# cvxgrp/qcqp

Measured on AMD Instinct MI355X. Metric: restarts x coord-sweeps / sec (improve COORD_DESCENT phase-2 sweeps, 2n^2 flops each; whole step timed), higher is better.
Workload: dtype f64

## Files before the change

### qcqp_amd/csrc/capi.hip

```cpp
#include <dlfcn.h>
#include <unistd.h>
#include <hip/hip_runtime.h>
#include <rccl/rccl.h>

#include <algorithm>
#include <cmath>
#include <cstdarg>
#include <cstdio>
#include <cstring>
#include <string>
#include <chrono>
#include <vector>

#include "../../include/qcqp_mi.h"
#include "kernels_impl.h"
#include "admm.h"
#include "admm_fused.h"
#include "cd_queue.h"
#include "cd_life.h"
#include "cd_small.h"
#include "sdr_small.h"
#include "gemm_pk.h"
#include "cd_general.h"
#include "cd_dense.h"
// ... 131 lines not shown
    double stream_limit = 16e9;
    double *dn_gp_pre = nullptr, *dn_tmp = nullptr;
    ncclComm_t comm = nullptr;
    int rank = 0, world = 1;
    double *d_comm = nullptr, *d_comm_big = nullptr;
    int64_t comm_big_cap = 0;
    long long *d_prof = nullptr;
    int cd_stage = 0;
    int64_t Xi_cap = 0;
    bool sdr_factor_resident = false;
    double ad_Minv_rho = 0.0;
    bool ad_Minv_device = false;
    const char *last_cd2_kernel = "";
    bool profile = false;
    int dbg = 0;
    char *af_work = nullptr;
    size_t af_work_cap = 0;
    bool ad_fused = true;
    int ad_fused_nt = 512;
    const char *last_admm_kernel = "";
    int last_admm_C = 0;
    long long af_prof[16] = {0};
    int cd_queue = 2;
    int *d_qnext = nullptr;
    bool q_prepared = false;
    CdLife *d_life = nullptr;
    int Kreal = 0;
    double fbound = 0.0;
    double *l2_scratch = nullptr; size_t l2_scratch_cap = 0;
    double *l2_D = nullptr, *l2_S = nullptr;
    int *l2_abort = nullptr;
    int *l2_cuslot = nullptr;
    double *l2_preslack = nullptr; int64_t l2_preslack_cap = 0;
    double *lr_L = nullptr, *lr_G = nullptr, *lr_U = nullptr; int lr_RB = 0;
    int life_version = 0;
    long long *d_life_prof = nullptr;
    int64_t *d_bestK_idx = nullptr; double *d_bestK_key = nullptr, *d_bestK_x = nullptr; int64_t bestK_cap = 0;
    bool cd_ref_order = false;
    bool force_generic = false;
    std::vector<int> last_st1, last_st2;
    char *sb_work = nullptr;
    size_t sb_work_cap = 0;
    std::vector<double> unit_d;
    char *ss_work = nullptr;
    size_t ss_work_cap = 0;
};

namespace {

void admm_free(qcqpmi_ctx *c, bool keep_zsolver);

int fail(qcqpmi_ctx *c, int code, const char *fmt, ...) {
    char buf[1024];
    va_list ap;
    va_start(ap, fmt);
    vsnprintf(buf, sizeof(buf), fmt, ap);
    va_end(ap);
    if (c) c->err = buf; else g_create_error = buf;
    return code;
}

#define HIPCHK(c, expr)                                                                       \
    do {                                                                                      \
        hipError_t e_ = (expr);                                                               \
        if (e_ != hipSuccess)                                                                 \
            return fail(c, QCQPMI_EHIP, "%s failed: %s (%s:%d)", #expr, hipGetErrorString(e_), \
// ... 463 lines not shown
    if (!out || n <= 0 || m < 0) return fail(nullptr, QCQPMI_EINVAL, "ctx_create: bad arguments");
    int ndev = qcqpmi_device_count();
    if (ndev <= 0)
        return fail(nullptr, QCQPMI_EHIP, "no HIP device visible: the qcqp_amd engine requires an MI355X (there is no CPU fallback)");
    if (device < 0 || device >= ndev) return fail(nullptr, QCQPMI_EINVAL, "device %d out of range (%d visible)", device, ndev);
    qcqpmi_ctx *c = new qcqpmi_ctx();
    c->device = device; c->n = n; c->m = m; c->n16 = (n + 15) / 16 * 16;
    c->quads.resize((size_t)m + 1);
    if (const char *sl = getenv("QCQPMI_STREAM_LIMIT")) { const double v = atof(sl); if (v > 0.0) c->stream_limit = v; }
    hipError_t e = hipSetDevice(device);
    if (e == hipSuccess) e = hipStreamCreateWithFlags(&c->stream, hipStreamNonBlocking);
    for (int i = 0; i < 5 && e == hipSuccess; i++) {
        e = hipEventCreate(&c->timers[i].beg);
        if (e == hipSuccess) e = hipEventCreate(&c->timers[i].end);
    }
    if (e != hipSuccess) {
        int rc = fail(nullptr, QCQPMI_EHIP, "ctx_create: %s", hipGetErrorString(e));
        delete c;
        return rc;
    }
    *out = c;
    return 0;
}

void qcqpmi_ctx_destroy(qcqpmi_ctx *c) {
    if (!c) return;
    (void)hipSetDevice(c->device);
    if (c->stream) (void)spin_sync(c->stream);
    if (c->comm && rccl() && rccl()->CommDestroy) rccl()->CommDestroy(c->comm);
    free_population(c);
    admm_free(c, false);
    for (void *p : c->prob_allocs) (void)hipFree(p);
    void *ptrs[] = {c->d_Fpack, c->d_Frow, c->d_mu, c->d_best_idx, c->d_best_key, c->d_comm, c->d_comm_big,
                    c->dn_G, c->dn_Dg, c->dn_Ft, c->dn_prof, c->dn_state, c->d_planes, c->d_out, c->d_wS, c->d_wY, c->d_ww, c->d_wz, c->af_work, c->d_qnext, c->d_life, c->d_life_prof, c->d_bestK_idx, c->d_bestK_key, c->d_bestK_x, c->l2_scratch, c->l2_D, c->l2_S, c->l2_abort, c->l2_cuslot, c->l2_preslack, c->lr_L, c->lr_G, c->lr_U, c->sb_work, c->ss_work};
    if (c->h_out) (void)hipHostFree(c->h_out);
    if (c->h_pin) (void)hipHostFree(c->h_pin);
    for (void *p : ptrs) if (p) (void)hipFree(p);
    for (auto &t : c->timers) { if (t.beg) (void)hipEventDestroy(t.beg); if (t.end) (void)hipEventDestroy(t.end); }
    for (auto &e : c->dn_ev) if (e) (void)hipEventDestroy(e);
    for (auto &e : c->dn_evn) if (e) (void)hipEventDestroy(e);
    if (c->dn_hn) (void)hipHostFree(c->dn_hn);
    if (c->stream2) (void)hipStreamDestroy(c->stream2);
    if (c->stream) (void)hipStreamDestroy(c->stream);
    delete c;
}

int qcqpmi_set_quad(qcqpmi_ctx *c, int64_t k, int format, const double *vals, const int64_t *idx,
                    const int64_t *ptr, int64_t nnz, const double *q, double r, int relop) {
    if (!c) return QCQPMI_EINVAL;
    if (c->finalized) return fail(c, QCQPMI_ESTATE, "set_quad after finalize");
    if (k < 0 || k > c->m || !q) return fail(c, QCQPMI_EINVAL, "set_quad: bad k or q");
    if ((k == 0) != (relop == 0) || relop < 0 || relop > 2)
        return fail(c, QCQPMI_EINVAL, "set_quad: relop %d invalid for function %lld", relop, (long long)k);
    HostQuad &h = c->quads[(size_t)k];
    h = HostQuad();
    const int64_t n = c->n;
    if (format == QCQPMI_FMT_DENSE) {
        if (!vals) return fail(c, QCQPMI_EINVAL, "set_quad: dense vals missing");
        for (int64_t i = 0; i < n; i++)
            for (int64_t j = 0; j < n; j++) {
                double v = vals[i * n + j];
                if (v != 0.0) { h.ci.push_back((int)i); h.cj.push_back((int)j); h.cv.push_back(v); }
            }
    } else if (format == QCQPMI_FMT_CSR) {
        if (!ptr || (nnz > 0 && (!idx || !vals))) return fail(c, QCQPMI_EINVAL, "set_quad: CSR arrays missing");
        for (int64_t i = 0; i < n; i++)
            for (int64_t e = ptr[i]; e < ptr[i + 1]; e++) {
// ... 693 lines not shown
    return qcqpmi_cd_run_stage(c, 0, phase1, num_iters, viol_tol, tol, seed, first_index, sweeps1, sweeps2, visits2, accepted2,
                               ran_phase2, f0, maxviol);
}

int qcqpmi_cd_dense_block_step(qcqpmi_ctx *c, int phase, int64_t sweep, int64_t block, int coord_lo, int coord_hi, double viol_tol,
                               double tol, uint64_t seed, uint64_t first_index, const double *slack) {
    int rc = check_ready(c, true);
    if (rc) return rc;
    if (!dense_on(c)) return fail(c, QCQPMI_EUNSUPPORTED, "cd_dense_block_step: the problem does not take the dense-constraint path");
    c->last_cd2_kernel = dense_chain_name(c);
    return cd_dense_block_step(c, phase, sweep, block, coord_lo, coord_hi, viol_tol, tol, seed, first_index, slack);
}

static int cd_life2_reserve(qcqpmi_ctx *c, int nmw, int cus) {
    int rc;
    const size_t need = (size_t)cd_life2_max_wgs(nmw, cus, 1) * (size_t)c->n16 * 16;
    if (need > c->l2_scratch_cap) {
        if (c->l2_scratch) { HIPCHK(c, spin_sync(c->stream)); (void)hipFree(c->l2_scratch); c->l2_scratch = nullptr; c->l2_scratch_cap = 0; }
        if ((rc = dev_alloc(c, &c->l2_scratch, need))) return rc;
        c->l2_scratch_cap = need;
    }
    if (!c->l2_abort && (rc = dev_alloc(c, &c->l2_abort, 4))) return rc;
    if (!c->l2_cuslot && (rc = dev_alloc(c, &c->l2_cuslot, 4096))) return rc;
    if (!c->l2_D) {
        const size_t NB = (size_t)(c->n16 / 16);
        if ((rc = dev_alloc(c, &c->l2_D, NB * 256))) return rc;
        if ((rc = dev_alloc(c, &c->l2_S, NB * 48))) return rc;
        hipError_t e = (hipError_t)cd_life2_pack(c->dp, c->l2_D, c->l2_S, c->stream);
        if (e != hipSuccess) return fail(c, QCQPMI_EHIP, "cd_life2_pack: %s", hipGetErrorString(e));
    }
    return 0;
}

int qcqpmi_cd_stream_run(qcqpmi_ctx *c, int64_t K, int64_t R, int generate, int phase1, int64_t num_iters, double viol_tol, double tol,
                         uint64_t seed, uint64_t seed_stride, uint64_t first_index, uint64_t first_stride, double select_tol,
                         int64_t *sweeps1, int64_t *sweeps2, int64_t *visits2, int64_t *accepted2, uint8_t *ran_phase2, double *f0,
                         double *maxviol, int64_t *best_index, double *best_f0, double *best_maxviol, double *best_x) {
    int rc = check_ready(c, generate ? false : true);
    if (rc) return rc;
    if (K < 1 || R < 1 || num_iters < 0 || !(tol > 0.0) || K * R >= (1LL << 30)) return fail(c, QCQPMI_EINVAL, "cd_stream_run: bad K / R / num_iters / tol");
    if (!generate && c->R != K * R) return fail(c, QCQPMI_EINVAL, "cd_stream_run: the resident population has %lld points, K R = %lld", (long long)c->R, (long long)(K * R));
    HIPCHK(c, hipSetDevice(c->device));
    const bool stt = getenv("QCQPMI_STREAM_TIMING") != nullptr;
    double stm[6] = {0, 0, 0, 0, 0, 0};
    auto stnow = []() { return std::chrono::duration<double, std::milli>(std::chrono::steady_clock::now().time_since_epoch()).count(); };
    stm[0] = stnow();
    int nmw = 0, cs2 = 0, kind = 0;
    const int factor_rb = (c->lr_RB > 0 && c->life_version != 3 && cd_life2_factor_ok(c->dp, 16 * (int64_t)c->lr_RB)) ? c->lr_RB : 0;
    bool use2 = c->life_version != 1 && !c->force_generic && !(c->dbg & 64) && c->sep &&
                cd_life2_config(c->dp, c->Kreal, c->objclass, c->symcls, factor_rb, &nmw, &cs2, &kind);
    int cs = 0;
    const int queue_switch = c->cd_queue;
    c->cd_queue = 2;
    const bool eligible = cd_queue_eligible(c, false) && (int)(c->n16 / 16) - 4 <= RQ_NSIMD * RQ_MAXU && c->n16 >= 48;
    c->cd_queue = queue_switch;
    const bool lr = use2 && factor_rb > 0 && nmw == 3 && (kind == L2_KIND_BAND || kind == L2_KIND_GEN);
    if (lr) cs2 = 0;
    if (!use2) {
        if (!eligible || c->life_version != 1)
            return fail(c, QCQPMI_EUNSUPPORTED, "cd_stream_run: the lifecycle kernel needs separable constraints -- at most four classes of coordinates, at most two constraints "
                        "per coordinate --, a diagonal of P0 that is positive everywhere or zero everywhere (a diagonal of mixed sign: ONE class with one constraint "
                        "per coordinate only; with several classes or two constraints per coordinate it runs the serial path), and 33 <= n <= 2304: use qcqpmi_cd_run "
                        "per population");
        const int NBq = (int)(c->n16 / 16);
        cs = (c->dbg & 128) ? ((c->dbg >> 8) & 7) : 4;
        cs = cs > RQ_CSMAX ? RQ_CSMAX : cs;
        if (cs >= NBq) cs = 0;
        cs &= ~1;
        if (NBq - cs > RQ_NSIMD * RQ_MAXU || NBq < 3) return fail(c, QCQPMI_EUNSUPPORTED, "cd_stream_run: n = %lld outside the range of cd_phase2_qs_kernel (n <= 1024, at least 3 blocks of 16)", (long long)c->n);
    }
    if (generate && (rc = pop_reserve(c, K * R))) return rc;
    if (!c->d_qnext && (rc = dev_alloc(c, &c->d_qnext, 16))) return rc;
    if (!c->d_life) HIPCHK(c, hipMalloc((void **)&c->d_life, sizeof(CdLife)));
    HIPCHK(c, hipMemsetAsync(c->d_qnext, 0, 16 * sizeof(int), c->stream));
    CdLife L;
    L.on = 1; L.generate = generate ? 1 : 0; L.phase1 = phase1 ? 1 : 0; L.Rtotal = K * R; L.Rpop = R;
    L.seed = seed; L.seed_stride = seed_stride; L.first_index = first_index; L.first_stride = first_stride; L.viol_tol = viol_tol;
    L.sweeps1 = c->d_sweeps1; L.status1 = c->d_status1; L.ran2 = c->d_flag;
    L.prof = nullptr;
    const char *pre_ev = getenv("QCQPMI_L2_PREBUILT");
    const bool pre = lr && !(pre_ev && atoi(pre_ev) == 0);
    L.prebuilt = pre ? 1 : 0; L.preslack = nullptr;
    if (pre) {
        if (K * R > c->l2_preslack_cap) {
            if (c->l2_preslack) { HIPCHK(c, spin_sync(c->stream)); (void)hipFree(c->l2_preslack); c->l2_preslack = nullptr; c->l2_preslack_cap = 0; }
            if ((rc = dev_alloc(c, &c->l2_preslack, (size_t)(K * R)))) return rc;
            c->l2_preslack_cap = K * R;
        }
        L.preslack = c->l2_preslack;
    }
    if (c->profile) {
        if (!c->d_life_prof) HIPCHK(c, hipMalloc((void **)&c->d_life_prof, 24 * sizeof(long long)));
        HIPCHK(c, hipMemsetAsync(c->d_life_prof, 0, 24 * sizeof(long long), c->stream));
        L.prof = c->d_life_prof;
    }
    HIPCHK(c, hipMemcpyAsync(c->d_life, &L, sizeof(L), hipMemcpyHostToDevice, c->stream));
    HIPCHK(c, spin_sync(c->stream));
    int cus = 0;
    HIPCHK(c, hipDeviceGetAttribute(&cus, hipDeviceAttributeMultiprocessorCount, c->device));
    stm[1] = stnow();
    if (use2) {
        if ((rc = cd_life2_reserve(c, nmw, cus))) return rc;
        if (!lr && (c->dbg & 128)) { const int k2 = (c->dbg >> 8) & 7; if (nmw == 3 && (k2 == 0 || k2 == 2 || k2 == 4) && k2 < (int)(c->n16 / 16)) cs2 = k2; }
        const int tiles = cd_life2_tiles(c->dp, nmw, cs2, K * R, cus, 0, lr ? 1 : 0);
        int64_t wgs = (K * R + 16 * tiles - 1) / (16 * tiles);
        const int maxw = cd_life2_max_wgs(nmw, cus, tiles);
        if (wgs > maxw) wgs = maxw;
        if (c->dbg & 1024) { const int lim = (c->dbg >> 12) & 1023; if (lim > 0 && wgs > lim) wgs = lim; }
        CdLife2Args qa;
        qa.P = c->dp; qa.num_iters = num_iters; qa.tol = tol; qa.life = c->d_life;
        cd_queue_fill_batch(c, qa.b, seed, first_index);
        qa.b.R = K * R;
        qa.scratch = c->l2_scratch; qa.Dpack = c->l2_D; qa.Spack = c->l2_S; qa.abort = c->l2_abort; qa.fbound = c->fbound;
        { const char *ev = getenv("QCQPMI_L2_ROT"); const int rot = ev ? atoi(ev) : (lr ? 2 : 0); qa.cuslot = rot ? c->l2_cuslot : nullptr; qa.rotmode = rot; }
        if (qa.cuslot) HIPCHK(c, hipMemsetAsync(c->l2_cuslot, 0, 4096 * sizeof(int), c->stream));
        qa.dbg = (c->dbg & 2048) ? 1 : 0;
        qa.Gpack = lr ? c->lr_G : nullptr; qa.Upack = lr ? c->lr_U : nullptr; qa.RB = lr ? c->lr_RB : 0;
        qa.nclass = c->Kreal;
        const double l0 = stnow();
        (void)hipEventRecord(c->timers[2].beg, c->stream);
        const double l1 = stnow();
        hipError_t qe = pre ? (hipError_t)cd_life2_prep_launch(c->dp, c->d_life, c->X, K * R, num_iters, tol, c->stream) : hipSuccess;
        if (qe == hipSuccess) qe = (hipError_t)cd_life2_launch(qa, nmw, cs2, kind, tiles, (int)wgs, c->stream);
        const double l2 = stnow();
        (void)hipEventRecord(c->timers[2].end, c->stream);
        c->timers[2].valid = true;
        if (qe != hipSuccess) return fail(c, QCQPMI_EHIP, "cd_stream_run: %s", hipGetErrorString(qe));
        c->last_cd2_kernel = cd_life2_name(nmw, kind, tiles, lr ? 1 : 0);
        int ab = 0;
        HIPCHK(c, spin_sync(c->stream));
        const double l3 = stnow();
        HIPCHK(c, hipMemcpyAsync(&ab, c->l2_abort, sizeof(int), hipMemcpyDeviceToHost, c->stream));
        const double l4 = stnow();
        HIPCHK(c, spin_sync(c->stream));
        if (stt) fprintf(stderr, "cd_stream_run launch (ms): reserve %.3f, event %.3f, launch call %.3f, event + spin wait %.3f, copy call %.3f, sync %.3f\n", l0 - stm[1], l1 - l0, l2 - l1, l3 - l2, l4 - l3, stnow() - l4);
        if (ab) {
            HIPCHK(c, hipMemsetAsync(c->l2_abort, 0, sizeof(int), c->stream));
            c->R = 0;
            return fail(c, QCQPMI_EHIP, "cd_stream_run: a wait inside cd_life_kernel ran into its watchdog (internal error; no results)");
        }
    } else {
        CdQueueArgs qa;
        qa.P = c->dp; qa.num_iters = num_iters; qa.tol = tol;
        qa.life = c->d_life; qa.life_on = 1;
        cd_queue_fill_batch(c, qa.b, seed, first_index);
        qa.b.R = K * R;
        (void)hipEventRecord(c->timers[2].beg, c->stream);
        hipError_t qe = (hipError_t)cd_queue_launch(qa, cs, cus, c->stream);
        (void)hipEventRecord(c->timers[2].end, c->stream);
        c->timers[2].valid = true;
        if (qe != hipSuccess) return fail(c, QCQPMI_EHIP, "cd_stream_run: %s", hipGetErrorString(qe));
        HIPCHK(c, spin_sync(c->stream));
        c->last_cd2_kernel = "cd_phase2_qs_kernel<lifecycle>";
    }
    c->cd_stage = 0;
// ... 181 lines not shown
    a.max_sweeps = max_sweeps; a.tol = tol; a.seed = seed; a.seed_stride = seed_stride; a.first_index = first_index;
    a.ticket = (int *)(w + oticket);
    a.V = (double *)(w + oV); a.primal = (double *)(w + opr); a.y = (double *)(w + oy); a.sweeps = (int64_t *)(w + osw); a.X = (double *)(w + oX);
    const int wgs = sdr_small_workgroups((int)n, B, c->device);
    if (wgs < 1) return fail(c, QCQPMI_EHIP, "sdr_small_batch: occupancy query failed: %s", hipGetErrorString((hipError_t)(-wgs)));
    const hipError_t qe = (hipError_t)sdr_small_launch(a, wgs, c->stream);
    if (qe != hipSuccess) return fail(c, QCQPMI_EHIP, "sdr_small_batch: %s", hipGetErrorString(qe));
    int flags[2] = {0, 0};
    HIPCHK(c, hipMemcpyAsync(flags, w + oticket, sizeof(flags), hipMemcpyDeviceToHost, c->stream));
    HIPCHK(c, spin_sync(c->stream));
    if (flags[1]) return fail(c, QCQPMI_EINVAL, "sdr_small_batch: an objective matrix P0_b is not symmetric (or holds a NaN)");
    if (V) HIPCHK(c, hipMemcpyAsync(V, a.V, (size_t)B * N * SDR_SMALL_K * 8, hipMemcpyDeviceToHost, c->stream));
    if (primal) HIPCHK(c, hipMemcpyAsync(primal, a.primal, (size_t)B * 8, hipMemcpyDeviceToHost, c->stream));
    if (y) HIPCHK(c, hipMemcpyAsync(y, a.y, (size_t)B * N * 8, hipMemcpyDeviceToHost, c->stream));
    if (sweeps) HIPCHK(c, hipMemcpyAsync(sweeps, a.sweeps, (size_t)B * 8, hipMemcpyDeviceToHost, c->stream));
    if (X && S > 0) HIPCHK(c, hipMemcpyAsync(X, a.X, (size_t)B * S * n * 8, hipMemcpyDeviceToHost, c->stream));
    HIPCHK(c, spin_sync(c->stream));
    return 0;
}

int qcqpmi_cd_stream_reserve(qcqpmi_ctx *c, int64_t K, int64_t R) {
    int rc = check_ready(c, false);
    if (rc) return rc;
    if (K < 1 || R < 1 || K * R >= (1LL << 30)) return fail(c, QCQPMI_EINVAL, "cd_stream_reserve: bad K / R");
    HIPCHK(c, hipSetDevice(c->device));
    if (K * R > c->Rcap) { if ((rc = pop_reserve(c, K * R))) return rc; }
    if ((rc = cd_outputs_reserve(c, K * R))) return rc;
    if ((rc = cd_bestK_reserve(c, K))) return rc;
    if (!c->d_qnext && (rc = dev_alloc(c, &c->d_qnext, 16))) return rc;
    if (!c->d_life) HIPCHK(c, hipMalloc((void **)&c->d_life, sizeof(CdLife)));
    {
        int nmw = 0, cs2 = 0, kind = 0, cus = 0;
        HIPCHK(c, hipDeviceGetAttribute(&cus, hipDeviceAttributeMultiprocessorCount, c->device));
        if (c->life_version != 1 && c->sep && cd_life2_config(c->dp, c->Kreal, c->objclass, c->symcls, c->lr_RB, &nmw, &cs2, &kind) && (rc = cd_life2_reserve(c, nmw, cus))) return rc;
    }
    return 0;
}

int qcqpmi_debug_life_profile(qcqpmi_ctx *c, int64_t *out16) {
    if (!c || !out16) return QCQPMI_EINVAL;
    for (int k = 0; k < 24; k++) out16[k] = 0;
    if (!c->d_life_prof) return 0;
    HIPCHK(c, hipSetDevice(c->device));
    HIPCHK(c, spin_sync(c->stream));
    HIPCHK(c, hipMemcpy(out16, c->d_life_prof, 24 * sizeof(long long), hipMemcpyDeviceToHost));
    return 0;
}

int qcqpmi_cd_status(qcqpmi_ctx *c, int *status1, int *status2) {
    if (!c) return QCQPMI_EINVAL;
    if ((int64_t)c->last_st1.size() != c->R || (int64_t)c->last_st2.size() != c->R)
        return fail(c, QCQPMI_ESTATE, "cd_status: no coordinate-descent run on the resident population");
    if (status1) memcpy(status1, c->last_st1.data(), (size_t)c->R * sizeof(int));
    if (status2) memcpy(status2, c->last_st2.data(), (size_t)c->R * sizeof(int));
    return 0;
}


int qcqpmi_select_best(qcqpmi_ctx *c, double tol, int64_t *best_index, double *best_f0,
                       double *best_maxviol, double *best_x) {
    int rc = check_ready(c, true);
    if (rc) return rc;
    HIPCHK(c, hipSetDevice(c->device));
    if (!c->evaluated && (rc = launch_eval(c, false))) return rc;
    hipLaunchKernelGGL(select_best_kernel, dim3(1), dim3(1024), 0, c->stream, c->d_f0, c->d_mv, c->R, tol,
                       c->d_best_idx, c->d_best_key);
    HIPCHK(c, hipGetLastError());
// ... 234 lines not shown
```

### qcqp_amd/csrc/cd_life.h

```cpp
#pragma once
#include <hip/hip_runtime.h>
#include <stdint.h>
#include "kernels.h"
#include "cd_queue.h"

namespace qcqpmi {

enum { L2_KIND_BAND = 0, L2_KIND_GEN = 1, L2_KIND_LIN = 2, L2_KIND_GENK = 3, L2_KIND_LINK = 4, L2_KIND_SGN = 5 };

struct CdLife2Args {
    DevProblem P;
    CdBatch b;
    int64_t num_iters;
    double tol;
    const CdLife *life;
    double *scratch;
    const double *Dpack;
    const double *Spack;
    int *abort;
    int *cuslot;
    double fbound;
    const double *Gpack, *Upack;
    int RB;
    int rotmode;
    int nclass;
    int dbg;
};

bool cd_life2_config(const DevProblem &P, int Kreal, int objclass, bool symcls, int factor_rb, int *nmw, int *cs, int *kind);
size_t cd_life2_lds_bytes(int nmw, int cs, int tiles, int lr, int kind);
bool cd_life2_factor_ok(const DevProblem &P, int64_t r);
int cd_life2_pack_factor(const double *Lrow, double *Gpack, double *Upack, int NB, int RB, hipStream_t st);
int cd_life2_max_wgs(int nmw, int cus, int tiles);
int cd_life2_tiles(const DevProblem &P, int nmw, int cs, int64_t restarts, int cus, int requested, int lr);
int cd_life2_pack(const DevProblem &P, double *Dpack, double *Spack, hipStream_t st);
int cd_life2_prep_launch(const DevProblem &P, const CdLife *life, double *X, int64_t Rtotal, int64_t num_iters, double tol, hipStream_t st);
int cd_life2_launch(const CdLife2Args &a, int nmw, int cs, int kind, int tiles, int wgs, hipStream_t st);
const char *cd_life2_name(int nmw, int kind, int tiles, int lr);

}
```

### qcqp_amd/csrc/cd_life.hip

```cpp
#include "cd_life.h"

#include <cstdio>
#include <cstdlib>

#include "onevar.h"
#include "cd_phase1_sep.h"
#include "cd_chain.h"
#include "cd_roles.h"

namespace qcqpmi {
namespace {

constexpr int L2_WD = 1 << 21;
enum { L2_ABORT = 3 };

__device__ __attribute__((always_inline)) inline RqOwn l2_own(int NB, int CS, int m, int NMW) {
    RqOwn o;
    const int rest = NB - CS;
    o.NB = NB;
    if (m < 0) { o.first = rest; o.stride = 1; o.nu = CS; }
    else { o.first = m; o.stride = NMW; o.nu = m < rest ? (rest - m + NMW - 1) / NMW : 0; }
    return o;
}

// ... 806 lines not shown
#pragma unroll
        for (int u = 0; u < 4; u++) { p1v[u] = ring[g1 * 256 + u * 64 + lane]; p0v[u] = ring[g0 * 256 + u * 64 + lane]; }
#pragma unroll
        for (int u = 0; u < 4; u++) { pend[u * 64 + lane] = p1v[u]; pend[256 + u * 64 + lane] = p0v[u]; }
    }
    rq_sync_write(sy, RQ_STOP, 1, lane);
    if (prof_on && lane == 0) {
        atomicAdd(pprof + 13, (unsigned long long)pt_sum);
        atomicAdd(pprof + 14, (unsigned long long)pt_steps);
        atomicAdd(pprof + 15, (unsigned long long)pt_end);
        atomicAdd(pprof + 19, (unsigned long long)pt_req);
        *(long long *)(ctl + 8) = (long long)__builtin_amdgcn_s_memtime();
        atomicAdd(pprof + 7, (unsigned long long)pt_fix);
        atomicAdd(pprof + 8, (unsigned long long)pw_part);
        atomicAdd(pprof + 11, (unsigned long long)pn_int);
        atomicAdd(pprof + 12, (unsigned long long)pn_gen);
    }
    {
        cst[0 * 64 + lane] = S.upd_counter; cst[1 * 64 + lane] = S.visits; cst[2 * 64 + lane] = S.accepted;
        cst[3 * 64 + lane] = S.sweeps; cst[4 * 64 + lane] = S.conv ? 1 : 0; cst[5 * 64 + lane] = S.status;
        cst[6 * 64 + lane] = __double_as_longlong(fpart);
        cst[7 * 64 + lane] = (frz ? 1 : 0) | (done ? 2 : 0) | (pre ? 4 : 0) | (ld ? 8 : 0);
        cst[8 * 64 + lane] = __double_as_longlong(facc);
        const double ftot = rq_quad_sum(facc) + P.r0;
        const bool fin = occupied && done;
        if (gq == 0) {
            sfin[r] = fin ? 1 : 0;
            if (fin) { ovis[r] = S.visits; oacc[r] = S.accepted; oswp[r] = S.sweeps; ost[r] = S.status; of0[r] = ftot; }
        }
    }
    __builtin_amdgcn_s_setprio(0);
}

template <int NMW, int CS, int KIND, int TILES, int LR>
__global__ __launch_bounds__((NMW == 3 && TILES == 1) ? 256 : 512, 2) void cd_life_kernel(CdLife2Args a0) {
    const CdLife2Args &a = a0;
    constexpr bool MULTI = KIND == L2_KIND_GENK || KIND == L2_KIND_LINK;
    constexpr int BK = KIND == L2_KIND_GENK ? L2_KIND_GEN : KIND == L2_KIND_LINK ? L2_KIND_LIN : KIND;
    constexpr int MAXC = MULTI ? 2 : 1;
    constexpr int KCLV = MULTI ? L2_KCL : 1;
    constexpr int CSU = CS > 0 ? CS : 1;
    constexpr int LRV = LR;
    static_assert(!MULTI || (TILES == 1 && !LR), "multi-class kinds: one tile per workgroup, no objective factor");
    constexpr int NT = (NMW == 3 && TILES == 1) ? 256 : 512;
    constexpr int NW = NT / 64;
    constexpr int NS = 16 * TILES;
    constexpr int TD = l2_tile_doubles(NMW, CSU, LR);
    static_assert(!LR || (NMW == 3 && CS == 0 && BK != L2_KIND_LIN && BK != L2_KIND_SGN), "factored objective: three multiplying waves per tile, no chain share, a positive diagonal");
    constexpr bool PRE = BK == L2_KIND_LIN || BK == L2_KIND_SGN;
    static_assert(TILES == 1 || NMW == 3, "two tiles per workgroup: eight waves = two chains + two x three multiplying waves");
    const DevProblem &P = a.P;
    const int tid0 = threadIdx.x;
    const int wave = __builtin_amdgcn_readfirstlane(tid0 >> 6);
    const int64_t n16 = P.n16;
    const int NB = (int)P.NB, KS = (int)P.KS;
    L2_LDS_VIEW(0)
    (void)fixp; (void)gtile; (void)DU2; (void)sc2; (void)ring; (void)cshare; (void)of0; (void)ovis; (void)oacc; (void)oswp; (void)ost; (void)ytile; (void)pend; (void)clsb;
#define L2_STORE_SETS(st_, sc_, slack_) {                                                                                              \
        SetTable<MAXC> T2 = TC;                                                                                                          \
        T2.lo = l2_tl(TC.lo, st_, TD); T2.hi = l2_tl(TC.hi, st_, TD); T2.n = l2_tl(TC.n, st_, TD); T2.slow = l2_tl(TC.slow, st_, TD);    \
        const int nk_ = MULTI ? a0.nclass : 1;                                                                                           \
        for (int k_ = 0; k_ < nk_; k_++) {                                                                                               \
            FeasSet<MAXC> C_;                                                                                                            \
            compute_set<MAXC>(P, P.krep[k_], slack_, C_);                                                                                \
            store_set<MAXC>(T2, 16 * k_ + (sc_), C_);                                                                                    \
            if (MULTI && C_.n > 2) T2.slow[16 * k_ + (sc_)] = 1;                                                                         \
// ... 68 lines not shown
        asm volatile("" : "+s"(lifep));
        const int lane = tid & 63, r = lane >> 2;
        if (tid == 0) { ctl[0] = 0; jn[0] = 0; jn[1] = 0; }
        __syncthreads();
        if (tid < NS) {
            const int st = tid >> 4, sc = tid & 15;
            int id = l2_tl(sid, st, TD)[sc], nw = 0;
            if (id < 0) {
                GLB const CdLife *lf = glb(lifep);
                const int idx = glb_add(glb(a0.b.next), 1);
                if (idx < (int)lf->Rtotal) {
                    id = idx; nw = 1;
                    const uint64_t pop = (uint64_t)idx / (uint64_t)lf->Rpop, rho = (uint64_t)idx % (uint64_t)lf->Rpop;
                    l2_tl(sseed, st, TD)[sc] = lf->seed + pop * lf->seed_stride;
                    l2_tl(sfirst, st, TD)[sc] = lf->first_index + pop * lf->first_stride + rho - (uint64_t)idx;
                }
            }
            l2_tl(sid, st, TD)[sc] = id; l2_tl(snew, st, TD)[sc] = nw;
            if (nw) { l2_tl(p1fin, st, TD)[sc] = 0; l2_tl(p1sw, st, TD)[sc] = 0; l2_tl(p1st, st, TD)[sc] = 0; l2_tl(gatep, st, TD)[sc] = 0; }
            if (id < 0) {
                l2_tl(slk, st, TD)[sc] = 0.0;
                L2_STORE_SETS(st, sc, 0.0)
            }
            if (id >= 0) atomicAdd(&ctl[0], 1);
            *(volatile rq_lds_int *)(l2_tl((int *)sy, st, TD) + sc) = (sc >= RQ_PARTS + NMW) ? 0x7fffffff : 0;
        }
        __syncthreads();
        if (ctl[0] == 0) break;
        {
            __builtin_amdgcn_s_setprio(3);
            GLB const CdLife *lf = glb(lifep);
            const long long pt0 = lf->prof ? (long long)__builtin_amdgcn_s_memtime() : 0;
            const int lf_pre = LR ? lf->prebuilt : 0;
            const int lf_generate = lf->generate && !lf_pre, lf_phase1 = lf->phase1 && !lf_pre;
            const double lf_viol_tol = lf->viol_tol;
            const int e0 = P.cptr[P.krep[0]];
            const double cp = P.cp[e0], cq = P.cq[e0], cr = P.cr[e0];
            const int rel = P.crel[e0];
            for (int c = 0; c < NS; c++) {
                const int ct = c >> 4, cc = c & 15;
                GLB double *Xg = Xg0 + (int64_t)ct * n16 * 16;
                if (!l2_tl(snew, ct, TD)[cc]) {
                    if (l2_tl(sid, ct, TD)[cc] < 0) for (int64_t j = tid; j < n16; j += NT) Xg[j * 16 + cc] = 0.0;
                    continue;
                }
                if (!lf_generate) {
                    const int id = l2_tl(sid, ct, TD)[cc];
                    GLB const double *src = glb(a0.b.X) + ((int64_t)(id >> 4) * n16) * 16 + (id & 15);
                    for (int64_t j0 = tid; j0 < n16; j0 += 4 * NT) {
                        double t4[4];
#pragma unroll
                        for (int u = 0; u < 4; u++) t4[u] = (j0 + u * NT < n16) ? src[(j0 + u * NT) * 16] : 0.0;
#pragma unroll
                        for (int u = 0; u < 4; u++) if (j0 + u * NT < n16) Xg[(j0 + u * NT) * 16 + cc] = t4[u];
                    }
                }
            }
            if (lf_generate) {
                if (tid == 0) {
                    int cnt = 0;
                    for (int k = 0; k < NS; k++) if (l2_tl(snew, k >> 4, TD)[k & 15]) p1cols[cnt++] = k;
                    ctl[4] = cnt; ctl[5] = 0;
                }
                __syncthreads();
                const int ncolg = ctl[4], nchg = (int)((n16 + 127) / 128);
                for (;;) {
// ... 113 lines not shown
                const int st = tid >> 4, sc = tid & 15;
                double mvx;
                if (lf_pre) {
                    const int id = l2_tl(sid, st, TD)[sc];
                    mvx = glb(lf->preslack)[id];
                    l2_tl(p1sw, st, TD)[sc] = (int)glb(lf->sweeps1)[id];
                    l2_tl(p1st, st, TD)[sc] = glb(lf->status1)[id];
                    l2_tl(gatep, st, TD)[sc] = glb(lf->ran2)[id];
                } else {
                    mvx = ordered_unkey(l2_tl(p1key, st, TD)[sc]);
                    l2_tl(gatep, st, TD)[sc] = (mvx < lf_viol_tol && l2_tl(p1st, st, TD)[sc] == 0) ? 1 : 0;
                }
                l2_tl(slk, st, TD)[sc] = mvx;
                L2_STORE_SETS(st, sc, mvx)
            }
            __syncthreads();
            if (nlast < 16) {
                for (int w = tid; w < NS * (16 - nlast); w += NT) {
                    const int c = w % NS, ct = c >> 4, cc = c & 15, row = w / NS;
                    if (l2_tl(snew, ct, TD)[cc] || l2_tl(sid, ct, TD)[cc] < 0) {
                        const int nn = l2_tl(TC.n, ct, TD)[cc];
                        double xp = 0.0;
                        if (BK == L2_KIND_BAND) xp = nn >= 2 ? l2_tl(TC.lo, ct, TD)[16 * KCLV + cc] : 0.0;
                        else if (BK == L2_KIND_GEN) xp = nn >= 1 ? l2_tl(TC.hi, ct, TD)[cc] : 0.0;
                        else xp = nn >= 2 ? l2_tl(TC.hi, ct, TD)[16 * KCLV + cc] : l2_tl(TC.hi, ct, TD)[cc];
                        if (!(xp == xp) || __builtin_isinf(xp)) xp = 0.0;
                        (Xg0 + (int64_t)ct * n16 * 16)[(P.n + row) * 16 + cc] = xp;
                    }
                }
                __syncthreads();
            }
            if (LR) {
                const int r16 = 16 * a0.RB;
                for (int w = tid; w < NS * (32 + r16); w += NT) {
                    const int c = w % NS, ct = c >> 4, cc = c & 15, rowz = w / NS;
                    if (l2_tl(snew, ct, TD)[cc] || l2_tl(sid, ct, TD)[cc] < 0) {
                        if (rowz < 32) l2_tl(pend, ct, TD)[rowz * 16 + cc] = 0.0;
                        else l2_tl(ytile, ct, TD)[(rowz - 32) * 16 + cc] = 0.0;
                    }
                }
                __syncthreads();
            }
            if (lf->prof && tid == 0) {
                int nn = 0;
                for (int k = 0; k < NS; k++) nn += l2_tl(snew, k >> 4, TD)[k & 15] ? 1 : 0;
                atomicAdd((unsigned long long *)lf->prof + 0, (unsigned long long)((long long)__builtin_amdgcn_s_memtime() - pt0));
                atomicAdd((unsigned long long *)lf->prof + 2, 1ull);
                atomicAdd((unsigned long long *)lf->prof + 3, (unsigned long long)nn);
            }
            __builtin_amdgcn_s_setprio(0);
        }
        if (role == 0) {
            long long *cs_ = l2_tl(cst, rtile, TD);
            if (l2_tl(snew, rtile, TD)[r]) {
#pragma unroll
                for (int f = 0; f < 6; f++) cs_[f * 64 + lane] = 0;
                const int pass = l2_tl(gatep, rtile, TD)[r];
                cs_[6 * 64 + lane] = 0;
                cs_[4 * 64 + lane] = (pass && !PRE && !LR) ? 0 : 1;
                cs_[7 * 64 + lane] = (pass ? (PRE ? 4 : 0) : 1) | (LR ? 8 : 0);
                cs_[8 * 64 + lane] = 0;
            } else if (l2_tl(sid, rtile, TD)[r] < 0) {
                cs_[4 * 64 + lane] = 1; cs_[6 * 64 + lane] = 0;
                cs_[7 * 64 + lane] = 2; cs_[8 * 64 + lane] = 0;
            }
        }
        __syncthreads();
        if (tid == 0 && glb(lifep)->prof) *(long long *)(ctl + 6) = (long long)__builtin_amdgcn_s_memtime();

        if (role > 0) {
            if (LR) l2_mfma_lr_role<NMW>(role - 1, rtile);
            else l2_mfma_role<NMW, CS>(role - 1, rtile);
        } else l2_chain_role<NMW, CS, KIND, TILES, LR>(rtile);

        __syncthreads();
        if (sy[L2_ABORT] || (TILES > 1 && l2_tl((int *)sy, 1, TD)[L2_ABORT])) {
            if (tid == 0) __hip_atomic_store(glb(a0.abort), 1, __ATOMIC_RELAXED, __HIP_MEMORY_SCOPE_AGENT);
            break;
        }
        if (tid == 0 && glb(lifep)->prof)
        {
            const long long now_ = (long long)__builtin_amdgcn_s_memtime();
            atomicAdd((unsigned long long *)glb(lifep)->prof + 5, (unsigned long long)(now_ - *(long long *)(ctl + 6)));
            atomicAdd((unsigned long long *)glb(lifep)->prof + 20, (unsigned long long)(now_ - *(long long *)(ctl + 8)));
        }
        {
            const int e0 = P.cptr[P.krep[0]];
            const double cp = P.cp[e0], cq = P.cq[e0], cr = P.cr[e0];
            const int rel = P.crel[e0];
            if (tid == 0) { int cnt = 0; for (int k = 0; k < NS; k++) if (l2_tl(sfin, k >> 4, TD)[k & 15]) p1cols[cnt++] = k; ctl[4] = cnt; }
            if (tid < NS) l2_tl(p1key, tid >> 4, TD)[tid & 15] = ordered_key(-QM_INF);
            __syncthreads();
            const int nfin = ctl[4];
// ... 133 lines not shown
            if (stv) st1[s] = stv;
            __syncthreads();
            if (tid < 16 && !fin[tid]) {
                sw[tid]++;
                if (ordered_unkey(key[tid]) < viol_tol || !upd[tid]) fin[tid] = 1;
            }
        }
    }
    __syncthreads();
    if (tid < 16) key[tid] = ordered_key(-QM_INF);
    __syncthreads();
    double v = -QM_INF;
    if (valid)
        for (int64_t j = 2 * g; j < n; j += 32)
            for (int64_t i = j; i < j + 2 && i < n; i++) {
                const double x = Xt[16 * i];
                const double f = (cp * x + cq) * x + cr;
                const double w = (rel == RELOP_EQ) ? fabs(f) : (f > 0.0 ? f : 0.0);
                v = w > v ? w : v;
            }
#pragma unroll
    for (int o = 16; o <= 32; o <<= 1) { const double w = __shfl_xor(v, o, 64); v = w > v ? w : v; }
    if ((tid & 63) < 16 && valid) atomicMax(&key[s], ordered_key(v));
    __syncthreads();
    if (tid < 16 && valid) {
        const double mvx = ordered_unkey(key[tid]);
        glb(const_cast<double *>(lf->preslack))[id] = mvx;
        glb(lf->sweeps1)[id] = sw[tid];
        glb(lf->status1)[id] = st1[tid];
        glb(lf->ran2)[id] = (mvx < viol_tol && st1[tid] == 0) ? 1 : 0;
    }
}

__global__ void l2_pack_kernel(DevProblem P, double *Dpack, double *Spack) {
    const int b = blockIdx.x, t = threadIdx.x;
    const int64_t n16 = P.n16;
    const int rr = t >> 4, cc = t & 15;
    Dpack[(int64_t)b * 256 + t] = (cc > rr) ? P.P0[(16 * (int64_t)b + rr) * n16 + 16 * b + cc] : 0.0;
    if (t < 16) {
        const int64_t i = 16 * (int64_t)b + t;
        const double d = P.P0[i * n16 + i], rc = P.rcp2d[i];
        Spack[(int64_t)b * 48 + t] = 0.5 * P.q0[i];
        Spack[(int64_t)b * 48 + 16 + t] = rc + rc;
        Spack[(int64_t)b * 48 + 32 + t] = d;
    }
}

__global__ void l2_pack_factor_kernel(const double *__restrict__ L, double *__restrict__ Gpack, double *__restrict__ Upack, int NB, int RB) {
    const int64_t idx = (int64_t)blockIdx.x * blockDim.x + threadIdx.x;
    if (idx >= (int64_t)NB * RB * 256) return;
    const int e = (int)(idx & 1), lane = (int)((idx >> 1) & 63), vp = (int)((idx >> 7) & 1);
    const int64_t rest = idx >> 8;
    const int beta = (int)(rest % RB), b = (int)(rest / RB), v = 2 * vp + e;
    const int64_t r16 = 16 * (int64_t)RB;
    Gpack[idx] = L[(16 * (int64_t)b + (lane & 15)) * r16 + 16 * beta + 4 * v + (lane >> 4)];
    Upack[idx] = L[(16 * (int64_t)b + 4 * v + (lane >> 4)) * r16 + 16 * beta + (lane & 15)];
}

template <int NMW, int CS, int TILES, int LR>
int l2_launch_kind(const CdLife2Args &a, int kind, int wgs, size_t lds, hipStream_t st) {
    constexpr bool MK = TILES == 1 && !LR;
    if (!MK && (kind == L2_KIND_GENK || kind == L2_KIND_LINK)) return (int)hipErrorInvalidValue;
    if (LR && kind == L2_KIND_SGN) return (int)hipErrorInvalidValue;
    auto k = kind == L2_KIND_SGN ? cd_life_kernel<NMW, CS, LR ? L2_KIND_GEN : L2_KIND_SGN, TILES, LR> : kind == L2_KIND_BAND ? cd_life_kernel<NMW, CS, L2_KIND_BAND, TILES, LR> : (kind == L2_KIND_GEN || LR) ? cd_life_kernel<NMW, CS, L2_KIND_GEN, TILES, LR>
             : kind == L2_KIND_GENK ? cd_life_kernel<NMW, CS, MK ? L2_KIND_GENK : L2_KIND_GEN, TILES, LR>
             : kind == L2_KIND_LINK ? cd_life_kernel<NMW, CS, MK ? L2_KIND_LINK : L2_KIND_GEN, TILES, LR>
                                    : cd_life_kernel<NMW, CS, LR ? L2_KIND_GEN : L2_KIND_LIN, TILES, LR>;
    hipError_t e = hipFuncSetAttribute((const void *)k, hipFuncAttributeMaxDynamicSharedMemorySize, (int)lds);
    if (e != hipSuccess) return (int)e;
    hipLaunchKernelGGL(k, dim3((unsigned)wgs), dim3((NMW == 3 && TILES == 1) ? 256 : 512), lds, st, a);
    return (int)hipGetLastError();
}

}

size_t cd_life2_lds_bytes(int nmw, int cs, int tiles, int lr, int kind) {
    const bool multi = kind == L2_KIND_GENK || kind == L2_KIND_LINK;
    return ((size_t)L2_SHARED_DOUBLES + (size_t)tiles * (size_t)l2_tile_doubles(nmw, cs > 0 ? cs : 1, lr, multi ? L2_KCL : 1, multi ? 2 : 1)) * sizeof(double) + 256;
}

bool cd_life2_factor_ok(const DevProblem &P, int64_t r) {
    const int64_t r16 = (r + 15) / 16 * 16;
    if (r < 1 || r16 > 16 * L2_YBMAX || P.NB < 8) return false;
    return true;
}

int cd_life2_pack_factor(const double *Lrow, double *Gpack, double *Upack, int NB, int RB, hipStream_t st) {
    const int64_t tot = (int64_t)NB * RB * 256;
    hipLaunchKernelGGL(l2_pack_factor_kernel, dim3((unsigned)((tot + 255) / 256)), dim3(256), 0, st, Lrow, Gpack, Upack, NB, RB);
    return (int)hipGetLastError();
}

int cd_life2_prep_launch(const DevProblem &P, const CdLife *life, double *X, int64_t Rtotal, int64_t num_iters, double tol, hipStream_t st) {
    hipLaunchKernelGGL(cd_life_prep_kernel, dim3((unsigned)((Rtotal + 15) / 16)), dim3(L2P_NT), 0, st, P, life, X, num_iters, tol);
    return (int)hipGetLastError();
}

int cd_life2_max_wgs(int nmw, int cus, int tiles) { return (nmw == 3 && tiles == 1) ? 2 * cus : cus; }

bool cd_life2_config(const DevProblem &P, int Kreal, int objclass, bool symcls, int factor_rb, int *nmw, int *cs, int *kind) {
    if (!P.sep || P.maxc < 1 || P.maxc > 2 || Kreal < 1 || Kreal > L2_KCL) return false;
    const bool multi = P.maxc > 1 || Kreal > 1;
    if (objclass != 0 && objclass != 1 && objclass != 2) return false;
    if (objclass == 0 && multi) return false;
    const int NB = (int)P.NB;
    if (NB < 3) return false;
    int w, c;
    if (NB <= 4) { w = 3; c = 0; }
    else if (NB - 4 <= 3 * RQ_MAXU) { w = 3; c = (NB < 8) ? 2 : 4; }
    else if (factor_rb > 0 && !multi && objclass == 1 && NB <= 256) { w = 3; c = 0; }
    else if (NB - 4 <= 7 * RQ_MAXU) { w = 7; c = 4; }
    else return false;
    *nmw = w; *cs = c;
    *kind = objclass == 0 ? L2_KIND_SGN : multi ? (objclass == 2 ? L2_KIND_LINK : L2_KIND_GENK) : objclass == 2 ? L2_KIND_LIN : (symcls ? L2_KIND_BAND : L2_KIND_GEN);
    return true;
}

int cd_life2_tiles(const DevProblem &P, int nmw, int cs, int64_t restarts, int cus, int requested, int lr) {
    (void)P; (void)restarts; (void)cus;
    if (!lr || nmw != 3 || cs != 0) return 1;
    int t = requested;
    if (const char *ev = getenv("QCQPMI_L2_TILES")) t = atoi(ev);
    return t == 2 ? 2 : 1;
}

int cd_life2_pack(const DevProblem &P, double *Dpack, double *Spack, hipStream_t st) {
    hipLaunchKernelGGL(l2_pack_kernel, dim3((unsigned)P.NB), dim3(256), 0, st, P, Dpack, Spack);
// ... 47 lines not shown
```

### qcqp_amd/csrc/cd_queue.h

```cpp
#pragma once
#include <hip/hip_runtime.h>
#include <stdint.h>
#include "kernels.h"

namespace qcqpmi {

struct CdBatch {
    double *X;
    const double *f0cur;
    const double *slack;
    const uint8_t *flag;
    int64_t *visits, *accepted, *sweeps;
    int *status;
    double *f0out, *mvout;
    int64_t R;
    uint64_t seed, first_index;
    int *next;
};

struct CdLife {
    int on;
    int generate;
    int phase1;
    int64_t Rtotal, Rpop;
    uint64_t seed, seed_stride, first_index, first_stride;
    double viol_tol;
    int64_t *sweeps1;
    int *status1;
    uint8_t *ran2;
    long long *prof;
    int prebuilt;
    const double *preslack;
};

struct CdQueueArgs {
    DevProblem P;
    CdBatch b;
    int64_t num_iters;
    double tol;
    const CdLife *life;
    int life_on;
};

size_t cd_queue_lds_bytes(const DevProblem &P);
int cd_queue_launch(const CdQueueArgs &a, int cs, int max_wgs, hipStream_t st);

}
```

Measured before the change: 28.16 million.

## Precompute low-rank factor projections y0 in a separate MFMA kernel before CD

Adds a pre-pass kernel that computes, for every restart tile, the initial low-rank factor projection Y0 = U^T x with f64 MFMA and stores it in a device buffer. The main coordinate-descent kernel then loads these precomputed columns into LDS when a new restart enters a slot, instead of computing them inline. This aims to take the per-restart setup projection off the persistent kernel's critical path. In exchange it costs an extra kernel launch, extra global memory (capped by an environment limit), and a global read per new restart.

```diff
diff --git a/qcqp_amd/csrc/capi.hip b/qcqp_amd/csrc/capi.hip
--- a/qcqp_amd/csrc/capi.hip
+++ b/qcqp_amd/csrc/capi.hip
@@ -187,6 +187,7 @@
     int *l2_abort = nullptr;
     int *l2_cuslot = nullptr;
     double *l2_preslack = nullptr; int64_t l2_preslack_cap = 0;
+    double *l2_y0 = nullptr; size_t l2_y0_cap = 0;
     double *lr_L = nullptr, *lr_G = nullptr, *lr_U = nullptr; int lr_RB = 0;
     int life_version = 0;
     long long *d_life_prof = nullptr;
@@ -716,7 +717,7 @@
     admm_free(c, false);
     for (void *p : c->prob_allocs) (void)hipFree(p);
     void *ptrs[] = {c->d_Fpack, c->d_Frow, c->d_mu, c->d_best_idx, c->d_best_key, c->d_comm, c->d_comm_big,
-                    c->dn_G, c->dn_Dg, c->dn_Ft, c->dn_prof, c->dn_state, c->d_planes, c->d_out, c->d_wS, c->d_wY, c->d_ww, c->d_wz, c->af_work, c->d_qnext, c->d_life, c->d_life_prof, c->d_bestK_idx, c->d_bestK_key, c->d_bestK_x, c->l2_scratch, c->l2_D, c->l2_S, c->l2_abort, c->l2_cuslot, c->l2_preslack, c->lr_L, c->lr_G, c->lr_U, c->sb_work, c->ss_work};
+                    c->dn_G, c->dn_Dg, c->dn_Ft, c->dn_prof, c->dn_state, c->d_planes, c->d_out, c->d_wS, c->d_wY, c->d_ww, c->d_wz, c->af_work, c->d_qnext, c->d_life, c->d_life_prof, c->d_bestK_idx, c->d_bestK_key, c->d_bestK_x, c->l2_scratch, c->l2_D, c->l2_S, c->l2_abort, c->l2_cuslot, c->l2_preslack, c->l2_y0, c->lr_L, c->lr_G, c->lr_U, c->sb_work, c->ss_work};
     if (c->h_out) (void)hipHostFree(c->h_out);
     if (c->h_pin) (void)hipHostFree(c->h_pin);
     for (void *p : ptrs) if (p) (void)hipFree(p);
@@ -1476,6 +1477,28 @@
     return 0;
 }
 
+static int cd_life2_reserve_prebuilt(qcqpmi_ctx *c, int64_t restarts, bool *preload) {
+    int rc;
+    if (restarts > c->l2_preslack_cap) {
+        if (c->l2_preslack) { HIPCHK(c, spin_sync(c->stream)); (void)hipFree(c->l2_preslack); c->l2_preslack = nullptr; c->l2_preslack_cap = 0; }
+        if ((rc = dev_alloc(c, &c->l2_preslack, (size_t)restarts))) return rc;
+        c->l2_preslack_cap = restarts;
+    }
+    *preload = false;
+    const char *ev = getenv("QCQPMI_L2_PRELOAD"), *mb = getenv("QCQPMI_L2_PRELOAD_MB");
+    const size_t need = (size_t)((restarts + 15) / 16) * (size_t)c->lr_RB * 256;
+    if ((ev && atoi(ev) == 0) || c->lr_RB < 1 || (double)need * sizeof(double) > (mb ? atof(mb) : 1024.0) * 1048576.0) return 0;
+    if (need > c->l2_y0_cap) {
+        if (c->l2_y0) { HIPCHK(c, spin_sync(c->stream)); (void)hipFree(c->l2_y0); c->l2_y0 = nullptr; c->l2_y0_cap = 0; }
+        void *v = nullptr;
+        if (hipMalloc(&v, need * sizeof(double)) != hipSuccess) { (void)hipGetLastError(); return 0; }
+        c->l2_y0 = (double *)v;
+        c->l2_y0_cap = need;
+    }
+    *preload = true;
+    return 0;
+}
+
 int qcqpmi_cd_stream_run(qcqpmi_ctx *c, int64_t K, int64_t R, int generate, int phase1, int64_t num_iters, double viol_tol, double tol,
                          uint64_t seed, uint64_t seed_stride, uint64_t first_index, uint64_t first_stride, double select_tol,
                          int64_t *sweeps1, int64_t *sweeps2, int64_t *visits2, int64_t *accepted2, uint8_t *ran_phase2, double *f0,
@@ -1525,13 +1548,12 @@
     const char *pre_ev = getenv("QCQPMI_L2_PREBUILT");
     const bool pre = lr && !(pre_ev && atoi(pre_ev) == 0);
     L.prebuilt = pre ? 1 : 0; L.preslack = nullptr;
+    bool preload = false;
+    L.preloaded = 0; L.y0 = nullptr;
     if (pre) {
-        if (K * R > c->l2_preslack_cap) {
-            if (c->l2_preslack) { HIPCHK(c, spin_sync(c->stream)); (void)hipFree(c->l2_preslack); c->l2_preslack = nullptr; c->l2_preslack_cap = 0; }
-            if ((rc = dev_alloc(c, &c->l2_preslack, (size_t)(K * R)))) return rc;
-            c->l2_preslack_cap = K * R;
-        }
+        if ((rc = cd_life2_reserve_prebuilt(c, K * R, &preload))) return rc;
         L.preslack = c->l2_preslack;
+        if (preload) { L.preloaded = 1; L.y0 = c->l2_y0; }
     }
     if (c->profile) {
         if (!c->d_life_prof) HIPCHK(c, hipMalloc((void **)&c->d_life_prof, 24 * sizeof(long long)));
@@ -1565,6 +1587,7 @@
         (void)hipEventRecord(c->timers[2].beg, c->stream);
         const double l1 = stnow();
         hipError_t qe = pre ? (hipError_t)cd_life2_prep_launch(c->dp, c->d_life, c->X, K * R, num_iters, tol, c->stream) : hipSuccess;
+        if (qe == hipSuccess && preload) qe = (hipError_t)cd_life2_y0_launch(c->X, c->lr_U, c->l2_y0, (int)(c->n16 / 16), c->lr_RB, c->n16, K * R, c->stream);
         if (qe == hipSuccess) qe = (hipError_t)cd_life2_launch(qa, nmw, cs2, kind, tiles, (int)wgs, c->stream);
         const double l2 = stnow();
         (void)hipEventRecord(c->timers[2].end, c->stream);
@@ -1812,7 +1835,14 @@
     {
         int nmw = 0, cs2 = 0, kind = 0, cus = 0;
         HIPCHK(c, hipDeviceGetAttribute(&cus, hipDeviceAttributeMultiprocessorCount, c->device));
-        if (c->life_version != 1 && c->sep && cd_life2_config(c->dp, c->Kreal, c->objclass, c->symcls, c->lr_RB, &nmw, &cs2, &kind) && (rc = cd_life2_reserve(c, nmw, cus))) return rc;
+        const int factor_rb = (c->lr_RB > 0 && c->life_version != 3 && cd_life2_factor_ok(c->dp, 16 * (int64_t)c->lr_RB)) ? c->lr_RB : 0;
+        if (c->life_version != 1 && c->sep && cd_life2_config(c->dp, c->Kreal, c->objclass, c->symcls, factor_rb, &nmw, &cs2, &kind)) {
+            if ((rc = cd_life2_reserve(c, nmw, cus))) return rc;
+            const char *pre_ev = getenv("QCQPMI_L2_PREBUILT");
+            bool preload = false;
+            if (factor_rb > 0 && nmw == 3 && (kind == L2_KIND_BAND || kind == L2_KIND_GEN) && !(pre_ev && atoi(pre_ev) == 0) &&
+                (rc = cd_life2_reserve_prebuilt(c, K * R, &preload))) return rc;
+        }
     }
     return 0;
 }
diff --git a/qcqp_amd/csrc/cd_life.h b/qcqp_amd/csrc/cd_life.h
--- a/qcqp_amd/csrc/cd_life.h
+++ b/qcqp_amd/csrc/cd_life.h
@@ -35,6 +35,7 @@
 int cd_life2_tiles(const DevProblem &P, int nmw, int cs, int64_t restarts, int cus, int requested, int lr);
 int cd_life2_pack(const DevProblem &P, double *Dpack, double *Spack, hipStream_t st);
 int cd_life2_prep_launch(const DevProblem &P, const CdLife *life, double *X, int64_t Rtotal, int64_t num_iters, double tol, hipStream_t st);
+int cd_life2_y0_launch(const double *X, const double *Upack, double *Y0, int NB, int RB, int64_t n16, int64_t Rtotal, hipStream_t st);
 int cd_life2_launch(const CdLife2Args &a, int nmw, int cs, int kind, int tiles, int wgs, hipStream_t st);
 const char *cd_life2_name(int nmw, int kind, int tiles, int lr);
 
diff --git a/qcqp_amd/csrc/cd_life.hip b/qcqp_amd/csrc/cd_life.hip
--- a/qcqp_amd/csrc/cd_life.hip
+++ b/qcqp_amd/csrc/cd_life.hip
@@ -862,6 +862,28 @@
     __builtin_amdgcn_s_setprio(0);
 }
 
+template <int NS>
+__device__ __attribute__((noinline)) void l2_preload_columns(int tid, int RB, int NB, int64_t n16, int td, const int *sid, const int *snew, double *ytile,
+                                                             double *pend, const double *y0, GLB const double *Xg0) {
+    typedef __attribute__((address_space(3))) double lds_d;
+    typedef __attribute__((address_space(3))) const int lds_ci;
+    constexpr int KM = 2 + L2_YBMAX;
+    const int c = tid % NS, ct = c >> 4, cc = c & 15, rg = tid / NS;
+    const int id = ((lds_ci *)l2_tl(sid, ct, td))[cc];
+    const bool nw = ((lds_ci *)l2_tl(snew, ct, td))[cc] != 0;
+    if (!nw && id >= 0) return;
+    GLB const double *ysrc = glb(y0) + ((int64_t)(id >> 4) * (16 * RB) + rg) * 16 + (id & 15);
+    GLB const double *xsrc = Xg0 + ((int64_t)ct * n16 + 16 * (int64_t)(NB - 2) + rg) * 16 + cc;
+    lds_d *yt = (lds_d *)l2_tl(ytile, ct, td) + rg * 16 + cc, *pd = (lds_d *)l2_tl(pend, ct, td) + rg * 16 + cc;
+    double pv[KM];
+#pragma unroll
+    for (int k = 0; k < KM; k++) pv[k] = (nw && k < 2 + RB) ? (k < 2 ? xsrc[k * 256] : ysrc[(k - 2) * 256]) : 0.0;
+#pragma unroll
+    for (int k = 0; k < KM; k++)
+        if (k < 2) pd[k * 256] = pv[k];
+        else if (k < 2 + RB) yt[(k - 2) * 256] = pv[k];
+}
+
 template <int NMW, int CS, int KIND, int TILES, int LR>
 __global__ __launch_bounds__((NMW == 3 && TILES == 1) ? 256 : 512, 2) void cd_life_kernel(CdLife2Args a0) {
     const CdLife2Args &a = a0;
@@ -996,6 +1018,7 @@
             GLB const CdLife *lf = glb(lifep);
             const long long pt0 = lf->prof ? (long long)__builtin_amdgcn_s_memtime() : 0;
             const int lf_pre = LR ? lf->prebuilt : 0;
+            const int lf_preload = lf_pre ? lf->preloaded : 0;
             const int lf_generate = lf->generate && !lf_pre, lf_phase1 = lf->phase1 && !lf_pre;
             const double lf_viol_tol = lf->viol_tol;
             const int e0 = P.cptr[P.krep[0]];
@@ -1175,6 +1198,9 @@
             }
             if (LR) {
                 const int r16 = 16 * a0.RB;
+                static_assert(!LR || NT == 16 * NS, "l2_preload_columns: sixteen row groups per slot");
+                if (lf_preload) l2_preload_columns<NS>(tid, a0.RB, NB, n16, TD, sid, snew, ytile, pend, lf->y0, Xg0);
+                else
                 for (int w = tid; w < NS * (32 + r16); w += NT) {
                     const int c = w % NS, ct = c >> 4, cc = c & 15, rowz = w / NS;
                     if (l2_tl(snew, ct, TD)[cc] || l2_tl(sid, ct, TD)[cc] < 0) {
@@ -1190,6 +1216,7 @@
                 atomicAdd((unsigned long long *)lf->prof + 0, (unsigned long long)((long long)__builtin_amdgcn_s_memtime() - pt0));
                 atomicAdd((unsigned long long *)lf->prof + 2, 1ull);
                 atomicAdd((unsigned long long *)lf->prof + 3, (unsigned long long)nn);
+                if (lf_preload) atomicAdd((unsigned long long *)lf->prof + 21, (unsigned long long)nn);
             }
             __builtin_amdgcn_s_setprio(0);
         }
@@ -1199,9 +1226,10 @@
 #pragma unroll
                 for (int f = 0; f < 6; f++) cs_[f * 64 + lane] = 0;
                 const int pass = l2_tl(gatep, rtile, TD)[r];
+                const bool load = LR && !(glb(lifep)->prebuilt && glb(lifep)->preloaded);
                 cs_[6 * 64 + lane] = 0;
-                cs_[4 * 64 + lane] = (pass && !PRE && !LR) ? 0 : 1;
-                cs_[7 * 64 + lane] = (pass ? (PRE ? 4 : 0) : 1) | (LR ? 8 : 0);
+                cs_[4 * 64 + lane] = (pass && !PRE && !load) ? 0 : 1;
+                cs_[7 * 64 + lane] = (pass ? (PRE ? 4 : 0) : 1) | (load ? 8 : 0);
                 cs_[8 * 64 + lane] = 0;
             } else if (l2_tl(sid, rtile, TD)[r] < 0) {
                 cs_[4 * 64 + lane] = 1; cs_[6 * 64 + lane] = 0;
@@ -1401,6 +1429,56 @@
     }
 }
 
+constexpr int L2Y_NT = 256, L2Y_T = 2, L2Y_U = (L2_YBMAX + 3) / 4;
+__global__ __launch_bounds__(L2Y_NT) void cd_life_y0_kernel(const double *__restrict__ X, const double *__restrict__ Upack, double *__restrict__ Y0,
+                                                            int NB, int RB, int64_t n16, int64_t tiles) {
+    const int lane = threadIdx.x & 63, w = __builtin_amdgcn_readfirstlane((int)threadIdx.x >> 6);
+    const int nu = RB > w ? (RB - w + 3) / 4 : 0;
+    const int64_t t0 = (int64_t)blockIdx.x * L2Y_T;
+    GLB const v2d_ *up = (GLB const v2d_ *)glb(Upack) + (int64_t)w * 128 + lane;
+    GLB const double *xt[L2Y_T];
+#pragma unroll
+    for (int t = 0; t < L2Y_T; t++) xt[t] = glb(X) + (t0 + t < tiles ? t0 + t : tiles - 1) * n16 * 16 + lane;
+    v4d_ y[L2Y_U][L2Y_T];
+#pragma unroll
+    for (int u = 0; u < L2Y_U; u++)
+#pragma unroll
+        for (int t = 0; t < L2Y_T; t++) y[u][t] = v4d_{0.0, 0.0, 0.0, 0.0};
+    for (int b = 0; b < NB - 2; b++) {
+        v2d_ aU[L2Y_U][2];
+        double bd[L2Y_T][4];
+#pragma unroll
+        for (int u = 0; u < L2Y_U; u++)
+            if (u < nu) {
+                aU[u][0] = up[((int64_t)b * RB + 4 * u) * 128];
+                aU[u][1] = up[((int64_t)b * RB + 4 * u) * 128 + 64];
+            }
+#pragma unroll
+        for (int t = 0; t < L2Y_T; t++)
+#pragma unroll
+            for (int v = 0; v < 4; v++) bd[t][v] = xt[t][b * 256 + v * 64];
+#pragma unroll
+        for (int v = 0; v < 4; v++)
+#pragma unroll
+            for (int u = 0; u < L2Y_U; u++)
+                if (u < nu) {
+#pragma unroll
+                    for (int t = 0; t < L2Y_T; t++) y[u][t] = __builtin_amdgcn_mfma_f64_16x16x4f64(aU[u][v >> 1][v & 1], bd[t][v], y[u][t], 0, 0, 0);
+                }
+    }
+#pragma unroll
+    for (int t = 0; t < L2Y_T; t++)
+        if (t0 + t < tiles) {
+            GLB double *yo = glb(Y0) + (t0 + t) * RB * 256 + (lane >> 4) * 16 + (lane & 15);
+#pragma unroll
+            for (int u = 0; u < L2Y_U; u++)
+                if (u < nu) {
+#pragma unroll
+                    for (int v = 0; v < 4; v++) yo[(16 * (w + 4 * u) + 4 * v) * 16] = y[u][t][v];
+                }
+        }
+}
+
 __global__ void l2_pack_kernel(DevProblem P, double *Dpack, double *Spack) {
     const int b = blockIdx.x, t = threadIdx.x;
     const int64_t n16 = P.n16;
@@ -1462,6 +1540,13 @@
 
 int cd_life2_prep_launch(const DevProblem &P, const CdLife *life, double *X, int64_t Rtotal, int64_t num_iters, double tol, hipStream_t st) {
     hipLaunchKernelGGL(cd_life_prep_kernel, dim3((unsigned)((Rtotal + 15) / 16)), dim3(L2P_NT), 0, st, P, life, X, num_iters, tol);
+    return (int)hipGetLastError();
+}
+
+int cd_life2_y0_launch(const double *X, const double *Upack, double *Y0, int NB, int RB, int64_t n16, int64_t Rtotal, hipStream_t st) {
+    if (NB < 3 || RB < 1 || RB > L2_YBMAX) return (int)hipErrorInvalidValue;
+    const int64_t tiles = (Rtotal + 15) / 16;
+    hipLaunchKernelGGL(cd_life_y0_kernel, dim3((unsigned)((tiles + L2Y_T - 1) / L2Y_T)), dim3(L2Y_NT), 0, st, X, Upack, Y0, NB, RB, n16, tiles);
     return (int)hipGetLastError();
 }
 
diff --git a/qcqp_amd/csrc/cd_queue.h b/qcqp_amd/csrc/cd_queue.h
--- a/qcqp_amd/csrc/cd_queue.h
+++ b/qcqp_amd/csrc/cd_queue.h
@@ -31,6 +31,8 @@
     long long *prof;
     int prebuilt;
     const double *preslack;
+    int preloaded;
+    const double *y0;
 };
 
 struct CdQueueArgs {
```

After: 28.16 million. No clear change (-0.0%).
